# giltchcity/orb_slam3_ros

Measured on AMD Instinct MI355X. Metric: frames/sec ORB extract+match (752×480, 1000 kp) at 1/2/4/8 GPU; % HBM roofline, higher is better.
Workload: dtype u8; 1 GPU; EuRoC-MH01-like stereo 752x480 (BASELINE config 2): ORBextractor L+R (nFeatures=1000, scale 1.2, 8 levels, FAST 20/7) + ComputeStereoMatches; width=752, height=480, allgather=False, pipelines=1, parallelism=frame-sharded x1

## Files before the change

### orb_slam3_ros_amd/csrc/orbfe_kernels.hip

```cpp
#pragma clang fp contract(off)
#include <hip/hip_runtime.h>
#include <float.h>
#include <math.h>
#include <stdint.h>

#include <type_traits>

#include "brief_pattern.h"
#include "glibc_sincosf.h"
#include "orbfe_types.h"
#include "stl_sort.h"

namespace orbfe {

#define SYNC() __syncthreads()
#define WAVE_SYNC()                                               \
    do {                                                          \
        __builtin_amdgcn_fence(__ATOMIC_RELEASE, "workgroup");    \
        __builtin_amdgcn_s_waitcnt(0xc07f);                       \
        __builtin_amdgcn_wave_barrier();                          \
        __builtin_amdgcn_fence(__ATOMIC_ACQUIRE, "workgroup");    \
    } while (0)

__constant__ int c_umax[16] = {15, 15, 15, 15, 14, 14, 14, 13, 13, 12, 11, 10, 9, 8, 6, 3};
// ... 753 lines not shown
                    *(bi ? s_ent + pos : trash) = (uint16_t)((packed + i) | 0x4000 | (di << 15));
                    pos += (int)bi;
                }
                nent = __builtin_amdgcn_readlane(incl, 63);
            }
            WAVE_SYNC();
            for (int j0 = 0; j0 < nent; j0 += 128) {
                const int j = j0 + 2 * lane;
                const uint32_t e2 = j < nent ? ((const uint32_t*)s_ent)[j >> 1] : 0u;
                const bool ok0 = j < nent, ok1 = j + 1 < nent;
                const uint32_t e0 = e2 & 0xFFFFu, e1 = ok1 ? e2 >> 16 : e0;
                const uint8_t* q0 = s_px + (((e0 >> 7) & 127) + 3) * RS + (e0 & 127) + 3;
                const uint8_t* q1 = s_px + (((e1 >> 7) & 127) + 3) * RS + (e1 & 127) + 3;
                const orbfe_half2 v2 = as_h2(__builtin_bit_cast(uint32_t, orbfe_ushort2{q0[0], q1[0]}));
                const uint32_t bmask = ((e0 & 0x4000u) ? 0x00008000u : 0u) | ((e1 & 0x4000u) ? 0x80000000u : 0u);
                const orbfe_half2 ns = as_h2(0xBC00BC00u ^ bmask);
                const orbfe_half2 sv = as_h2(h2_bits(v2) ^ bmask);
                const uint8_t* t0 = q0 - 3 * RS - 3;
                const uint8_t* t1 = q1 - 3 * RS - 3;
                orbfe_half2 P[16];
#pragma unroll
                for (int k = 0; k < 16; k++) {
                    const int o = (kRingDy[k] + 3) * RS + kRingDx[k] + 3;
                    const orbfe_half2 x2 = as_h2(__builtin_bit_cast(uint32_t, orbfe_ushort2{t0[o], t1[o]}));
                    P[k] = __builtin_elementwise_fma(x2, ns, sv);
                }
                orbfe_half2 m3[16], m9[16];
#pragma unroll
                for (int k = 0; k < 16; k++) m3[k] = hmin(hmin(P[k], P[(k + 1) & 15]), P[(k + 2) & 15]);
#pragma unroll
                for (int k = 0; k < 16; k++) m9[k] = hmin(hmin(m3[k], m3[(k + 3) & 15]), m3[(k + 6) & 15]);
                orbfe_half2 r[6];
#pragma unroll
                for (int k = 0; k < 5; k++) r[k] = hmax(hmax(m9[3 * k], m9[3 * k + 1]), m9[3 * k + 2]);
                r[5] = m9[15];
                const orbfe_half2 mx = hmax(hmax(hmax(r[0], r[1]), r[2]), hmax(hmax(r[3], r[4]), r[5]));
                const uint32_t mb = h2_bits(mx);
                const int bx = (mb & 0x8000u) ? -1 : (int)(mb & 0x7fffu);
                const int by = (mb & 0x80000000u) ? -1 : (int)((mb >> 16) & 0x7fffu);
                const bool c0 = ok0 && bx > th, c1 = ok1 && by > th;
                if (c0) s_sc[(((e0 >> 7) & 127) + 1) * RS + (e0 & 127) + 1] = (uint8_t)(bx - 1);
                if (c1) s_sc[(((e1 >> 7) & 127) + 1) * RS + (e1 & 127) + 1] = (uint8_t)(by - 1);
                const int cc = (int)c0 + (int)c1;
                const unsigned long long b0 = __ballot(cc & 1), b1 = __ballot(cc & 2);
                int pos = ncorner + lanes_below(b0) + 2 * lanes_below(b1);
                if (c0) s_cor[pos++] = (uint16_t)(e0 & 0x3FFFu);
                if (c1) s_cor[pos] = (uint16_t)(e1 & 0x3FFFu);
                ncorner += __popcll(b0) + 2 * __popcll(b1);
            }
            WAVE_SYNC();
        }
        nsurv = 0;
        for (int i0 = 0; i0 < ncorner; i0 += 64) {
            const int i = i0 + lane;
            bool surv = false;
            int p = 0, sc = 0;
            if (i < ncorner) {
                p = s_cor[i];
                const uint8_t* q = s_sc + ((p >> 7) + 1) * RS + (p & 127) + 1;
                const int n0 = q[-RS - 1], n1 = q[-RS], n2 = q[-RS + 1], n3 = q[-1], n4 = q[1];
                const int n5 = q[RS - 1], n6 = q[RS], n7 = q[RS + 1];
                sc = q[0];
                const int mx = max(max(max(n0, n1), max(n2, n3)), max(max(n4, n5), max(n6, n7)));
                surv = sc > mx;
            }
            const unsigned long long m = __ballot(surv);
            if (surv)
                out[nsurv + lanes_below(m)] = (uint32_t)(xr0 + (p & 127)) | ((uint32_t)(yr0 + (p >> 7)) << 12) |
                                              ((uint32_t)sc << 24);
            nsurv += __popcll(m);
        }
        if (nsurv > 0) break;
        WAVE_SYNC();
    }
    if (lane == 0) cellcnt[(size_t)b * g.total_cells + c] = nsurv;
    WAVE_SYNC();
}

#define FAST_WPB 1
__global__ __launch_bounds__(64 * FAST_WPB) void k_fast(const uint8_t* const* imgs, int in_pitch, const uint8_t* pyr,
                                              int pyr_stride, OrbGeom g, FastLds fl, uint32_t* cellkeys,
                                              int* cellcnt, int c_lo, int c_hi, int cpw) {
    extern __shared__ __attribute__((aligned(16))) uint8_t smem_fast[];
    const int wave = __builtin_amdgcn_readfirstlane(threadIdx.x >> 6), lane = lane_id();
    const int lb = xcd_logical(block_linear(), gridDim.x * gridDim.y);
    const int bx = lb % gridDim.x, b = lb / gridDim.x;
    uint8_t* s_img = smem_fast + wave * fl.wave_bytes;
    uint8_t* s_sc = s_img + fl.roi;
    uint16_t* s_cor = (uint16_t*)(s_sc + fl.sc);
    uint16_t* s_ent = (uint16_t*)((uint8_t*)s_cor + fl.cor);
    const int cbeg = c_lo + (bx * FAST_WPB + wave) * cpw;
    if (cbeg >= c_hi) return;
    const int cend = min(cbeg + cpw, c_hi);
    orbfe_u32x4 pf[FAST_PF];
    FastCell cur = fast_cell(imgs, in_pitch, pyr, pyr_stride, g, b, cbeg);
    fast_prefetch(cur, lane, pf);
    for (int c = cbeg; c < cend; c++) {
        int ng, nd, cpr, rpl;
        fast_geom(cur, &ng, &nd, &cpr, &rpl);
        const int dw = cur.cols - 6, dh = cur.rows - 6;
        fast_stage_cell(cur, pf, s_img, s_sc, lane);
        const FastCell me = cur;
        if (c + 1 < cend) {
            cur = fast_cell_next(cur, imgs, in_pitch, pyr, pyr_stride, g, b);
            fast_prefetch(cur, lane, pf);
        }
        if (fast_rsd(nd) == 12)
            fast_cell_detect<12>(g, fl, me, ng, nd, dw, dh, s_img, s_sc, s_cor, s_ent, cellkeys, cellcnt, b, c, lane);
        else
            fast_cell_detect<0>(g, fl, me, ng, nd, dw, dh, s_img, s_sc, s_cor, s_ent, cellkeys, cellcnt, b, c, lane);
    }
}

#define OCT_NT 256
#define OCT_U 4
struct ExpLess64 {
    __device__ bool operator()(const unsigned long long& a, const unsigned long long& b) const {
        return (a >> 32) < (b >> 32);
    }
};
__device__ __forceinline__ int quadrant(uint32_t key, int x0, int x1, int y0, int y1) {
    const int halfX = (int)ceilf((float)(x1 - x0) / 2.f);
    const int halfY = (int)ceilf((float)(y1 - y0) / 2.f);
    const float fx = (float)(key & 0xfff), fy = (float)((key >> 12) & 0xfff);
    const int q = (fx < (float)(x0 + halfX)) ? (fy < (float)(y0 + halfY) ? 0 : 2) : (fy < (float)(y0 + halfY) ? 1 : 3);
    return q;
}
__device__ __forceinline__ void child_rect(int q, int x0, int x1, int y0, int y1, int* cx0, int* cx1, int* cy0,
                                           int* cy1) {
    const int mx = x0 + (int)ceilf((float)(x1 - x0) / 2.f);
    const int my = y0 + (int)ceilf((float)(y1 - y0) / 2.f);
    *cx0 = (q & 1) ? mx : x0;
    *cx1 = (q & 1) ? x1 : mx;
    *cy0 = (q & 2) ? my : y0;
    *cy1 = (q & 2) ? y1 : my;
}
template <int NT>
__device__ __forceinline__ int block_excl_scan(int* arr, int n, int* s_ws) {
    const int lane = lane_id(), wave = threadIdx.x >> 6;
    int carry = 0;
    for (int base = 0; base < n; base += NT) {
        const int i = base + threadIdx.x;
        const int v = i < n ? arr[i] : 0;
        const int incl = wave_incl_scan_dpp(v);
        if (lane == 63) s_ws[wave] = incl;
        SYNC();
        int woff = 0, tot = 0;
#pragma unroll
        for (int w = 0; w < NT / 64; w++) {
            const int t = s_ws[w];
            woff += w < wave ? t : 0;
            tot += t;
        }
        if (i < n) arr[i] = carry + woff + incl - v;
        carry += tot;
        SYNC();
    }
    return carry;
}

template <int NT>
__device__ __forceinline__ void block_scan2(int a, int b, int2* s_w2, int& exa, int& exb, int& tota, int& totb) {
    const int lane = lane_id(), wave = threadIdx.x >> 6;
    const int ia = wave_incl_scan_dpp(a), ib = wave_incl_scan_dpp(b);
    if (lane == 63) s_w2[wave] = make_int2(ia, ib);
    SYNC();
    int oa = 0, ob = 0, ta = 0, tb = 0;
#pragma unroll
    for (int w = 0; w < NT / 64; w++) {
        const int2 t = s_w2[w];
        oa += w < wave ? t.x : 0;
        ob += w < wave ? t.y : 0;
        ta += t.x;
        tb += t.y;
    }
    exa = oa + ia - a;
    exb = ob + ib - b;
    tota = ta;
    totb = tb;
}

__device__ __forceinline__ int wave_scan_lds(int* arr, int n) {
    const int lane = lane_id();
    int carry = 0;
    for (int base = 0; base < n; base += 64) {
        const int i = base + lane;
        const int v = i < n ? arr[i] : 0;
        const int incl = wave_incl_scan_dpp(v);
        if (i < n) arr[i] = carry + incl - v;
        carry += __builtin_amdgcn_readlane(incl, 63);
    }
    WAVE_SYNC();
    return carry;
}

__device__ __forceinline__ void atomic_inc_runs(int* base, int t, bool act) {
    const int lane = lane_id();
    const int key = act ? t : -1 - lane;
    const int prev = __builtin_amdgcn_update_dpp(INT_MIN, key, 0x138, 0xf, 0xf, false);
    const bool head = key != prev;
    const unsigned long long hm = __ballot(head);
    const unsigned long long above = hm & ~((2ull << lane) - 1ull);
    const int next = above ? (int)__builtin_ctzll(above) : 64;
    if (head && act) atomicAdd(&base[t], next - lane);
}

__device__ __forceinline__ int wave_partition(unsigned long long* a, int lo, int hi, int* lpos, int* rpos) {
    const int tid = lane_id();
    const unsigned long long lt = (1ull << tid) - 1ull;
    unsigned long long xpiv;
    {
        const int ia = lo + 1, ib = lo + (hi - lo) / 2, ic = hi - 1;
        const unsigned long long x0 = a[lo], xa = a[ia], xb = a[ib], xc = a[ic];
        const ExpLess64 comp;
        int pick;
        if (comp(xa, xb)) pick = comp(xb, xc) ? ib : (comp(xa, xc) ? ic : ia);
        else pick = comp(xa, xc) ? ia : (comp(xb, xc) ? ic : ib);
        xpiv = pick == ia ? xa : (pick == ib ? xb : xc);
        if (tid == 0) {
            a[lo] = xpiv;
            a[pick] = x0;
        }
    }
    WAVE_SYNC();
    const unsigned P = (unsigned)(xpiv >> 32);
    const int m = hi - lo - 1;
    int* lp = lpos + lo;
    int* rp = rpos + lo;
    int nl = 0, nr = 0;
    for (int b0 = 0; b0 < m; b0 += 64) {
        const int i = b0 + tid;
        bool lf = false, rf = false;
        if (i < m) {
            lf = !((unsigned)(a[lo + 1 + i] >> 32) < P);
            rf = !(P < (unsigned)(a[hi - 1 - i] >> 32));
        }
        const unsigned long long lm = __ballot(lf), rm = __ballot(rf);
        if (lf) lp[nl + __popcll(lm & lt)] = lo + 1 + i;
        if (rf) rp[nr + __popcll(rm & lt)] = hi - 1 - i;
        nl += __popcll(lm);
        nr += __popcll(rm);
    }
    WAVE_SYNC();
    const int kmax = min(nl, nr);
    int sw = 0;
    for (int b0 = 0; b0 < kmax; b0 += 64) {
        const int k = b0 + tid;
        sw += __popcll(__ballot(k < kmax && lp[k] < rp[k]));
    }
    for (int k = tid; k < sw; k += 64) {
        const unsigned long long x = a[lp[k]];
        a[lp[k]] = a[rp[k]];
        a[rp[k]] = x;
    }
    int cut;
    if (sw == 0) cut = lp[0];
    else cut = (sw < nl && lp[sw] < rp[sw - 1]) ? lp[sw] : rp[sw - 1];
    WAVE_SYNC();
    return cut;
}

__device__ __forceinline__ void wave_leaf(unsigned long long* a, int lo, int hi) {
    const int lane = lane_id();
    const int len = hi - lo;
    if (len <= 1) return;
    if (len > 16) {
        if (lane == 0) st_heap_sort(a + lo, len, ExpLess64());
        WAVE_SYNC();
        return;
    }
    const unsigned long long x = a[lo + min(lane, len - 1)];
    const unsigned kx = (unsigned)(x >> 32);
    int r = 0;
#pragma unroll
    for (int u = 0; u < 16; u++) {
        const unsigned ku = (unsigned)__builtin_amdgcn_readlane((int)kx, u);
        r += (u < len && (ku < kx || (ku == kx && u < lane))) ? 1 : 0;
    }
    WAVE_SYNC();
    if (lane < len) a[lo + r] = x;
    WAVE_SYNC();
}

#if ORBFE_OCT_STAMPS
__device__ unsigned long long g_sort_ts[16 * 16 + 16];
__shared__ unsigned long long s_dbg_ts[16 * 16 + 16];
#endif
__device__ __forceinline__ unsigned long long rl64(unsigned long long x, int l) {
    const unsigned lo = (unsigned)__builtin_amdgcn_readlane((int)(unsigned)x, l);
    const unsigned hi = (unsigned)__builtin_amdgcn_readlane((int)(unsigned)(x >> 32), l);
    return ((unsigned long long)hi << 32) | lo;
}
__device__ __forceinline__ unsigned long long bp64(unsigned long long x, int src) {
    const unsigned lo = (unsigned)__builtin_amdgcn_ds_bpermute(src << 2, (int)(unsigned)x);
    const unsigned hi = (unsigned)__builtin_amdgcn_ds_bpermute(src << 2, (int)(unsigned)(x >> 32));
    return ((unsigned long long)hi << 32) | lo;
}
__device__ __forceinline__ unsigned long long pm64(unsigned long long x, int dst) {
    const unsigned lo = (unsigned)__builtin_amdgcn_ds_permute(dst << 2, (int)(unsigned)x);
    const unsigned hi = (unsigned)__builtin_amdgcn_ds_permute(dst << 2, (int)(unsigned)(x >> 32));
    return ((unsigned long long)hi << 32) | lo;
}

__device__ __forceinline__ void wave_sort64(unsigned long long* a, int lo0, int len, int d0) {
    const int lane = lane_id();
#if ORBFE_OCT_STAMPS
    int s64i = 0;
#define S64_STAMP() do { if (lane == 0 && s64i < 15 && (threadIdx.x >> 6) == 0 && blockIdx.x == 0 && blockIdx.y == 0) s_dbg_ts[256 + s64i] = __builtin_amdgcn_s_memtime(); s64i++; } while (0)
#else
#define S64_STAMP() do { } while (0)
#endif
    S64_STAMP();
    unsigned long long x = a[lo0 + min(lane, len - 1)];
    const unsigned long long below = (1ull << lane) - 1ull;
    const unsigned long long above = lane == 63 ? 0ull : (~0ull << (lane + 1));
    unsigned long long leafm = 0, heapm = 0;
    int sg_lo = 0, sg_hi = lane == 0 ? len : 0, sg_dp = lane == 0 ? d0 : 0;
    int sp = 1;
    while (sp > 0) {
        --sp;
        const int lo = __builtin_amdgcn_readlane(sg_lo, sp), hi = __builtin_amdgcn_readlane(sg_hi, sp);
        const int dp = __builtin_amdgcn_readlane(sg_dp, sp);
        if (hi - lo <= 16 || dp == 0) {
            leafm |= 1ull << lo;
            if (hi - lo > 16) heapm |= 1ull << lo;
            continue;
        }
        const int ia = lo + 1, ib = lo + (hi - lo) / 2, ic = hi - 1;
        const unsigned kx = (unsigned)(x >> 32);
        const unsigned ka = (unsigned)__builtin_amdgcn_readlane((int)kx, ia);
        const unsigned kb = (unsigned)__builtin_amdgcn_readlane((int)kx, ib);
        const unsigned kc = (unsigned)__builtin_amdgcn_readlane((int)kx, ic);
        int pick;
        if (ka < kb) pick = kb < kc ? ib : (ka < kc ? ic : ia);
        else pick = ka < kc ? ia : (kb < kc ? ic : ib);
        const unsigned long long x0 = rl64(x, lo), xp = rl64(x, pick);
        if (lane == lo) x = xp;
        else if (lane == pick) x = x0;
        const unsigned P = (unsigned)(xp >> 32);
        const unsigned k = (unsigned)(x >> 32);
        const bool inr = lane > lo && lane < hi;
        const bool lf = inr && !(k < P), rf = inr && !(P < k);
        const unsigned long long LM = __ballot(lf), RM = __ballot(rf);
        const int rl = __popcll(LM & below), rr = __popcll(RM & above);
        const bool sL = lf && __popcll(RM & above) > rl;
        const int sw = __popcll(__ballot(sL));
        const bool sR = rf && rr < sw;
        int cut;
        if (sw == 0) {
            cut = __builtin_ctzll(LM);
        } else {
            const int rp = __builtin_ctzll(__ballot(rf && rr == sw - 1));
            const int lp = sw < __popcll(LM) ? __builtin_ctzll(__ballot(lf && rl == sw)) : 64;
            cut = lp < rp ? lp : rp;
            const unsigned long long vR = pm64(x, sR ? rr : 63);
            const unsigned long long vL = pm64(x, sL ? rl : 63);
            const unsigned long long fromR = bp64(vR, rl & 63), fromL = bp64(vL, rr & 63);
            if (sL) x = fromR;
            else if (sR) x = fromL;
        }
        if (lane == sp) { sg_lo = cut; sg_hi = hi; sg_dp = dp - 1; }
        if (lane == sp + 1) { sg_lo = lo; sg_hi = cut; sg_dp = dp - 1; }
        sp += 2;
        S64_STAMP();
    }
    S64_STAMP();
    const unsigned long long upto = leafm & ~above;
    const int ls = 63 - __builtin_clzll(upto | 1ull);
    const unsigned long long after = leafm & above;
    const int le = after ? __builtin_ctzll(after) : len;
    const bool heap = (heapm >> ls) & 1ull;
    const unsigned kx = (unsigned)(x >> 32);
    unsigned kj[16];
#pragma unroll
    for (int u = 0; u < 16; u++) kj[u] = (unsigned)__builtin_amdgcn_ds_bpermute(min(ls + u, 63) << 2, (int)kx);
    int r = 0;
#pragma unroll
    for (int u = 0; u < 16; u++) {
        const int j = ls + u;
        r += (int)((j < le) & ((kj[u] < kx) | ((kj[u] == kx) & (j < lane))));
    }
    x = pm64(x, (lane < len && !heap) ? ls + r : lane);
    if (lane < len) a[lo0 + lane] = x;
    if (heapm) {
        WAVE_SYNC();
        if (lane == 0) {
            unsigned long long hm = heapm;
            while (hm) {
                const int hs = __builtin_ctzll(hm);
                hm &= hm - 1ull;
                const unsigned long long nx = leafm & (hs == 63 ? 0ull : (~0ull << (hs + 1)));
                const int he = nx ? __builtin_ctzll(nx) : len;
                st_heap_sort(a + lo0 + hs, he - hs, ExpLess64());
            }
        }
    }
    WAVE_SYNC();
    S64_STAMP();
#if ORBFE_OCT_STAMPS
    if (lane == 0 && (threadIdx.x >> 6) == 0 && blockIdx.x == 0 && blockIdx.y == 0) s_dbg_ts[256 + 15] = s64i;
#endif
#undef S64_STAMP
}

__device__ __forceinline__ void wave_sort_seg(unsigned long long* a, int lo0, int hi0, int dp0, int* lpos, int* rpos) {
    const int tid = lane_id();
    int sg_lo = lo0, sg_hi = tid == 0 ? hi0 : 0, sg_dp = tid == 0 ? dp0 : 0;
    int sp = 1;
    while (sp > 0) {
        --sp;
        const int lo = __builtin_amdgcn_readlane(sg_lo, sp), hi = __builtin_amdgcn_readlane(sg_hi, sp);
        const int depth = __builtin_amdgcn_readlane(sg_dp, sp);
        if (hi - lo <= 64 && depth > 0) {
            if (hi - lo > 1) wave_sort64(a, lo, hi - lo, depth);
            continue;
        }
        if (depth == 0) {
            wave_leaf(a, lo, hi);
            continue;
        }
        const int cut = wave_partition(a, lo, hi, lpos, rpos);
        if (tid == sp) { sg_lo = cut; sg_hi = hi; sg_dp = depth - 1; }
        if (tid == sp + 1) { sg_lo = lo; sg_hi = cut; sg_dp = depth - 1; }
        sp += 2;
    }
}

__device__ __forceinline__ unsigned long long seg_pack(int lo, int hi, int d) {
    return (unsigned long long)(unsigned)lo | ((unsigned long long)(unsigned)hi << 16) | ((unsigned long long)d << 32);
}

__device__ __forceinline__ void block_introsort(unsigned long long* a, int n, int* fl, int* lpos, int* rpos, int* leaves,
                                unsigned long long* tmp, int4* segs, int* s_ws, int* s_ctl) {
    (void)fl; (void)leaves; (void)segs; (void)s_ws;
    const int lane = lane_id(), wave = threadIdx.x >> 6, nw = blockDim.x >> 6;
#if ORBFE_OCT_STAMPS
    int sti = 0;
#define SORT_STAMP() do { if (lane == 0 && sti < 15 && blockIdx.x == 0 && blockIdx.y == 0) s_dbg_ts[wave * 16 + sti] = __builtin_amdgcn_s_memtime(); sti++; } while (0)
#else
#define SORT_STAMP() do { } while (0)
#endif
    SORT_STAMP();
    if (threadIdx.x == 0) {
        tmp[0] = seg_pack(0, n, 2 * st_lg(n));
#pragma unroll
        for (int k = 0; k < 8; k++) s_ctl[k] = 0;
    }
    SYNC();
    SORT_STAMP();
    if (n <= 1) return;
    unsigned long long* cur = tmp;
    unsigned long long* nxt = tmp + 2 * nw;
    int S = 1, r = 0;
    while (S > 0 && S < nw && r < 7) {
        bool any = false;
        for (int s = wave; s < S; s += nw) {
            const unsigned long long e = cur[s];
            const int lo = (int)(e & 0xffff), hi = (int)((e >> 16) & 0xffff), d = (int)(e >> 32);
            unsigned long long c0 = 0, c1 = 0;
            if (hi - lo <= 16 || d == 0) {
                wave_leaf(a, lo, hi);
            } else if (hi - lo <= 64) {
                wave_sort64(a, lo, hi - lo, d);
            } else {
                const int cut = wave_partition(a, lo, hi, lpos, rpos);
                if (hi - cut <= 16 || d == 1) wave_leaf(a, cut, hi);
                else c0 = seg_pack(cut, hi, d - 1);
                if (cut - lo <= 16 || d == 1) wave_leaf(a, lo, cut);
                else c1 = seg_pack(lo, cut, d - 1);
            }
            if (lane == 0) {
                nxt[2 * s] = c0;
                nxt[2 * s + 1] = c1;
            }
            any = any || c0 != 0 || c1 != 0;
        }
        if (any && lane == 0) s_ctl[r] = 1;
        SYNC();
        SORT_STAMP();
        S = s_ctl[r] ? 2 * S : 0;
        r++;
        unsigned long long* t = cur; cur = nxt; nxt = t;
    }
    for (int s = wave; s < S; s += nw) {
        const unsigned long long e = cur[s];
        if (e) wave_sort_seg(a, (int)(e & 0xffff), (int)((e >> 16) & 0xffff), (int)(e >> 32), lpos, rpos);
    }
    SORT_STAMP();
    SYNC();
    SORT_STAMP();
#if ORBFE_OCT_STAMPS
    if (lane == 0 && blockIdx.x == 0 && blockIdx.y == 0) s_dbg_ts[wave * 16 + 15] = sti;
    SYNC();
    if (blockIdx.x == 0 && blockIdx.y == 0)
        for (int i = threadIdx.x; i < 16 * 16 + 16; i += blockDim.x) g_sort_ts[i] = s_dbg_ts[i];
#endif
#undef SORT_STAMP
}

__global__ __launch_bounds__(OCT_NT) void k_debug_block_sort(unsigned long long* a, int n) {
    extern __shared__ __attribute__((aligned(16))) uint8_t smem_dbs[];
    unsigned long long* la = (unsigned long long*)smem_dbs;
    unsigned long long* tmp = la + n;
    int* fl = (int*)(tmp + n);
    int* lpos = fl + n;
    int* rpos = lpos + n;
    int* leaves = rpos + n;
    int4* segs = (int4*)(((uintptr_t)(leaves + n) + 15) & ~(uintptr_t)15);
    __shared__ int s_ws[OCT_NT / 64];
    __shared__ int s_ctl[8];
    for (int i = threadIdx.x; i < n; i += OCT_NT) la[i] = a[i];
    SYNC();
    block_introsort(la, n, fl, lpos, rpos, leaves, tmp, segs, s_ws, s_ctl);
    for (int i = threadIdx.x; i < n; i += OCT_NT) a[i] = la[i];
}

template <int NT>
__global__ __launch_bounds__(NT, NT <= 256 ? 6 : 1) void k_octree(OrbGeom g, const uint32_t* __restrict__ cellkeys,
                                                   const int* __restrict__ cellcnt, uint32_t* lkeys,
                                                   uint16_t* nodeof, uint32_t* outkeys, int* lvinfo, int* ranks,
                                                   const int2* __restrict__ laps, unsigned long long* tstamp,
                                                   int lv0) {
    extern __shared__ __attribute__((aligned(16))) uint8_t smem_oct[];
    const int b = blockIdx.x, l = lv0 + (int)blockIdx.y, tid = threadIdx.x;
    const int lap0 = laps[b].x, lap1 = laps[b].y;
    const OrbLevel& L = g.lv[l];
    const int NC = g.node_cap;
    const int ncell = L.n_cols * L.n_rows;
    uint8_t* p = smem_oct;
    auto carve = [&](size_t bytes) { uint8_t* r = p; p += (bytes + 15) & ~(size_t)15; return r; };
    int* cellpre = (int*)carve(sizeof(int) * (g.max_cells_level + 1));
    int16_t *Cx0 = (int16_t*)carve(2 * NC), *Cx1 = (int16_t*)carve(2 * NC);
    int16_t *Cy0 = (int16_t*)carve(2 * NC), *Cy1 = (int16_t*)carve(2 * NC);
    int* Csz = (int*)carve(4 * NC);
    int16_t *Xx0 = (int16_t*)carve(2 * NC), *Xx1 = (int16_t*)carve(2 * NC);
    int16_t *Xy0 = (int16_t*)carve(2 * NC), *Xy1 = (int16_t*)carve(2 * NC);
    int* Xsz = (int*)carve(4 * NC);
    int* Ccnt = (int*)carve(16 * NC);
    int* Xcnt = (int*)carve(16 * NC);
    int16_t* childpos = (int16_t*)carve(8 * NC);
    int16_t* newpos = (int16_t*)carve(2 * NC);
    int* divorder = (int*)carve(4 * NC);
    int* tmpA = (int*)carve(4 * NC);
    int* tmpB = (int*)carve(4 * NC);
    int* tmpC = (int*)carve(4 * NC);
    int* procp = (int*)carve(4 * NC);
    unsigned long long* expv = (unsigned long long*)carve(8 * NC);
    int4* segs = (int4*)carve(sizeof(int4) * ORBFE_SORT_STACK);
    __shared__ int s_ws[NT / 64];
    __shared__ int s_misc[8];
    __shared__ int2 s_ws2[NT / 64];

    unsigned long long* ts = (tstamp && b == 0) ? tstamp + 64 * l : nullptr;
    int tsi = 0;
    (void)ts;
    (void)tsi;
#if ORBFE_OCT_STAMPS
    __shared__ unsigned long long s_octts[64];
#define OCT_STAMP() do { if (ts && tid == 0 && tsi < 62) s_octts[tsi] = __builtin_amdgcn_s_memtime(); tsi++; } while (0)
#else
#define OCT_STAMP() do { } while (0)
#endif
    OCT_STAMP();
    const int* cc = cellcnt + (size_t)b * g.total_cells + L.cell_base;
    for (int i = tid; i < ncell; i += NT) cellpre[i] = cc[i];
    SYNC();
    const int K = block_excl_scan<NT>(cellpre, ncell, s_ws);
    if (tid == 0) cellpre[ncell] = K;
    const int nIni = L.n_ini;
    const float hX = L.hx;
    const int H = (L.h - ORBFE_MINB) - ORBFE_MINB;
    const bool fini = NT >= 1024 && K <= NT * (NT >= 1024 ? 8 : OCT_U) && nIni <= NT;
    for (int i = tid; i < nIni; i += NT) tmpA[i] = 0;
    if (fini)
        for (int i = tid; i < 4 * nIni; i += NT) tmpC[i] = 0;
    for (int i = tid; i < 4 * NC; i += NT) Ccnt[i] = 0;
    SYNC();
    const size_t kbase = (size_t)b * g.cellkeys_per_img + L.cellkey_off;
    uint32_t* keys = lkeys + kbase;
    uint16_t* nof = nodeof + kbase;
    const uint32_t* ck = cellkeys + kbase;
    constexpr int OU = NT >= 1024 ? 8 : OCT_U;
    const bool regk = NT >= 1024 && K <= NT * OU;
    uint32_t rkv[OU];
    int rq[OU];
    for (int kb = 0; kb < K; kb += NT * OU) {
        const int k0 = kb + tid;
        uint32_t v[OU];
#pragma unroll
        for (int u = 0; u < OU; u++) {
            if ((u & 3) == 0 && kb + NT * u >= K) break;
            const int k = min(k0 + NT * u, K - 1);
            int lo = 0, hi = ncell - 1;
            while (lo < hi) {
                const int mid = (lo + hi + 1) >> 1;
                if (cellpre[mid] <= k) lo = mid; else hi = mid - 1;
            }
            v[u] = ck[(size_t)lo * L.cell_cap + (k - cellpre[lo])];
        }
#pragma unroll
        for (int u = 0; u < OU; u++) {
            if ((u & 3) == 0 && kb + NT * u >= K) break;
            if (regk) rkv[u] = v[u];
            else if (k0 + NT * u < K) keys[k0 + NT * u] = v[u];
            const int col = (int)((float)(v[u] & 0xfff) / hX);
            atomic_inc_runs(tmpA, col, k0 + NT * u < K);
            if (fini) {
                rq[u] = col;
                atomic_inc_runs(tmpC, 4 * col + quadrant(v[u], (int)(hX * (float)col), (int)(hX * (float)(col + 1)), 0, H),
                                k0 + NT * u < K);
            }
        }
    }
    OCT_STAMP();
    SYNC();
    int n;
    if (fini) {
        const int i = tid;
        const bool f = i < nIni && tmpA[i] > 0;
        int ex, exZ, totZ;
        block_scan2<NT>(f ? 1 : 0, 0, s_ws2, ex, exZ, n, totZ);
        (void)exZ;
        (void)totZ;
        if (f) {
            Cx0[ex] = (int16_t)(int)(hX * (float)i);
            Cx1[ex] = (int16_t)(int)(hX * (float)(i + 1));
            Cy0[ex] = 0;
            Cy1[ex] = (int16_t)H;
            Csz[ex] = tmpA[i];
            *(int4*)&Ccnt[4 * ex] = *(const int4*)&tmpC[4 * i];
        }
        if (i < nIni) tmpB[i] = ex;
        for (int j = tid; j < NC; j += NT) divorder[j] = -1;
        SYNC();
#pragma unroll
        for (int u = 0; u < (NT >= 1024 ? 8 : OCT_U); u++) {
            if ((u & 3) == 0 && NT * u >= K) break;
            rq[u] = tmpB[rq[u]];
        }
        OCT_STAMP();
    } else {
    for (int i = tid; i < nIni; i += NT) tmpB[i] = tmpA[i] > 0 ? 1 : 0;
    SYNC();
    n = block_excl_scan<NT>(tmpB, nIni, s_ws);
    for (int i = tid; i < nIni; i += NT) {
        if (tmpA[i] > 0) {
            const int q = tmpB[i];
            Cx0[q] = (int16_t)(int)(hX * (float)i);
            Cx1[q] = (int16_t)(int)(hX * (float)(i + 1));
            Cy0[q] = 0;
            Cy1[q] = (int16_t)H;
            Csz[q] = tmpA[i];
        }
    }
    SYNC();
    for (int kb = 0; kb < K; kb += NT * OU) {
        const int k0 = kb + tid;
        uint32_t v[OU];
#pragma unroll
        for (int u = 0; u < OU; u++) v[u] = regk ? rkv[u] : keys[min(k0 + NT * u, K - 1)];
#pragma unroll
        for (int u = 0; u < OU; u++) {
            if ((u & 3) == 0 && kb + NT * u >= K) break;
            const int k = k0 + NT * u;
            const uint32_t key = v[u];
            const int q = tmpB[(int)((float)(key & 0xfff) / hX)];
            if (regk) rq[u] = q;
            else if (k < K) nof[k] = (uint16_t)q;
            atomic_inc_runs(Ccnt, 4 * q + quadrant(key, Cx0[q], Cx1[q], Cy0[q], Cy1[q]), k < K && Csz[q] > 1);
        }
    }
    for (int i = tid; i < NC; i += NT) divorder[i] = -1;
    SYNC();
    OCT_STAMP();
    }

    const int N = L.budget;
    bool phase2 = false, finish = false;
    int m = 0;
    int guard = 0;
    while (!finish && guard++ < 100000) {
        const int prevN = n;
        int newN, Etot;
        if (!phase2 && n <= NT) {
            const int i = tid;
            const bool live = i < n;
            const int csz = live ? Csz[i] : 0;
            const bool div = csz > 1;
            int4 cq = make_int4(0, 0, 0, 0);
            if (div) cq = *(const int4*)&Ccnt[4 * i];
            const int cv[4] = {cq.x, cq.y, cq.z, cq.w};
            int c = 0, e = 0;
#pragma unroll
            for (int k = 0; k < 4; k++) { c += cv[k] > 0; e += cv[k] > 1; }
            int exA, exB, totA, totB;
            block_scan2<NT>(live ? (div ? 1 : 0x10000) : 0, c | (e << 16), s_ws2, exA, exB, totA, totB);
            const int Ctot = totB & 0xffff;
            Etot = totB >> 16;
            newN = Ctot + (totA >> 16);
            if (div) {
                divorder[i] = exA & 0xffff;
                const int start = Ctot - ((exB & 0xffff) + c);
                int kk = 0;
                const int px0 = Cx0[i], px1 = Cx1[i], py0 = Cy0[i], py1 = Cy1[i];
                int cpos[4];
#pragma unroll
                for (int ch = 3; ch >= 0; ch--) {
                    const int v = cv[ch];
                    cpos[ch] = -1;
                    if (v > 0) {
                        const int np = start + kk++;
                        cpos[ch] = np;
                        childpos[4 * i + ch] = (int16_t)np;
                        int a0, a1, b0, b1;
                        child_rect(ch, px0, px1, py0, py1, &a0, &a1, &b0, &b1);
                        Xx0[np] = (int16_t)a0; Xx1[np] = (int16_t)a1;
                        Xy0[np] = (int16_t)b0; Xy1[np] = (int16_t)b1;
                        Xsz[np] = v;
                    } else {
                        childpos[4 * i + ch] = -1;
                    }
                }
                int ei = exB >> 16;
#pragma unroll
                for (int ch = 0; ch < 4; ch++) {
                    const int v = cv[ch];
                    if (v > 1) {
                        int a0, a1, b0, b1;
                        child_rect(ch, px0, px1, py0, py1, &a0, &a1, &b0, &b1);
                        expv[ei] = ((unsigned long long)v << 44) | ((unsigned long long)(a0 & 0xfff) << 32) |
                                   (unsigned long long)(uint16_t)cpos[ch];
                        ei++;
                    }
                }
            } else if (live) {
                divorder[i] = -1;
                const int np = Ctot + (exA >> 16);
                newpos[i] = (int16_t)np;
                Xx0[np] = Cx0[i]; Xx1[np] = Cx1[i];
                Xy0[np] = Cy0[i]; Xy1[np] = Cy1[i];
                Xsz[np] = csz;
            }
            for (int j = tid; j < 4 * newN; j += NT) Xcnt[j] = 0;
            SYNC();
            OCT_STAMP();
        } else if (phase2 && m <= NT && n <= NT) {
#if ORBFE_OCT_STAMPS
            if (ts && tid == 0) s_octts[62] = (unsigned long long)m | ((unsigned long long)n << 16) | ((unsigned long long)K << 32);
#endif
            block_introsort(expv, m, tmpC, tmpA, tmpB, Xcnt + 2 * NC, (unsigned long long*)Xcnt, segs, s_ws,
                            s_misc);
            OCT_STAMP();
            const int t = tid;
            const bool live = t < m;
            int q = 0;
            int4 cq = make_int4(0, 0, 0, 0);
            if (live) {
                q = (int)(expv[m - 1 - t] & 0xffffffffull);
                cq = *(const int4*)&Ccnt[4 * q];
            }
            const int cv[4] = {cq.x, cq.y, cq.z, cq.w};
            int c = 0, e = 0;
#pragma unroll
            for (int k = 0; k < 4; k++) { c += cv[k] > 0; e += cv[k] > 1; }
            const int grow = live ? c - 1 : 0;
            if (tid == 0) s_misc[6] = m;
            int exG, exCE, totG, totCE;
            block_scan2<NT>(grow, c | (e << 16), s_ws2, exG, exCE, totG, totCE);
            if (live && n + exG + grow >= N) atomicMin(&s_misc[6], t + 1);
            if (live) tmpB[t] = exCE + (c | (e << 16));
            SYNC();
            const int T_div = s_misc[6];
            const int tot = T_div > 0 ? tmpB[T_div - 1] : 0;
            const int Ctot = tot & 0xffff;
            Etot = tot >> 16;
            if (t < T_div) {
                divorder[q] = t;
                const int start = Ctot - ((exCE & 0xffff) + c);
                int kk = 0;
                const int px0 = Cx0[q], px1 = Cx1[q], py0 = Cy0[q], py1 = Cy1[q];
                int cpos[4];
#pragma unroll
                for (int ch = 3; ch >= 0; ch--) {
                    const int v = cv[ch];
                    cpos[ch] = -1;
                    if (v > 0) {
                        const int np = start + kk++;
                        cpos[ch] = np;
                        childpos[4 * q + ch] = (int16_t)np;
                        int a0, a1, b0, b1;
                        child_rect(ch, px0, px1, py0, py1, &a0, &a1, &b0, &b1);
                        Xx0[np] = (int16_t)a0; Xx1[np] = (int16_t)a1;
                        Xy0[np] = (int16_t)b0; Xy1[np] = (int16_t)b1;
                        Xsz[np] = v;
                    } else {
                        childpos[4 * q + ch] = -1;
                    }
                }
                int ei = exCE >> 16;
#pragma unroll
                for (int ch = 0; ch < 4; ch++) {
                    const int v = cv[ch];
                    if (v > 1) {
                        int a0, a1, b0, b1;
                        child_rect(ch, px0, px1, py0, py1, &a0, &a1, &b0, &b1);
                        expv[ei] = ((unsigned long long)v << 44) | ((unsigned long long)(a0 & 0xfff) << 32) |
                                   (unsigned long long)(uint16_t)cpos[ch];
                        ei++;
                    }
                }
            }
            SYNC();
            const int i = tid;
            const bool keep = i < n && divorder[i] < 0;
            int exK, exZ, nKeep, totZ;
            block_scan2<NT>(keep ? 1 : 0, 0, s_ws2, exK, exZ, nKeep, totZ);
            (void)exZ;
            (void)totZ;
            if (keep) {
                const int np = Ctot + exK;
                newpos[i] = (int16_t)np;
                Xx0[np] = Cx0[i]; Xx1[np] = Cx1[i];
                Xy0[np] = Cy0[i]; Xy1[np] = Cy1[i];
                Xsz[np] = Csz[i];
            }
            newN = Ctot + nKeep;
            for (int j = tid; j < 4 * newN; j += NT) Xcnt[j] = 0;
            SYNC();
            OCT_STAMP();
        } else {
            int T_div;
            if (!phase2) {
                for (int i = tid; i < n; i += NT) tmpA[i] = Csz[i] > 1 ? 1 : 0;
                SYNC();
                for (int i = tid; i < n; i += NT) divorder[i] = Csz[i] > 1 ? 1 : -1;
                T_div = block_excl_scan<NT>(tmpA, n, s_ws);
                for (int i = tid; i < n; i += NT)
                    if (divorder[i] >= 0) { divorder[i] = tmpA[i]; procp[tmpA[i]] = i; }
                SYNC();
            } else {
#if ORBFE_OCT_STAMPS
                if (ts && tid == 0) s_octts[62] = (unsigned long long)m | ((unsigned long long)n << 16) | ((unsigned long long)K << 32);
#endif
                block_introsort(expv, m, tmpC, tmpA, tmpB, Xcnt + 2 * NC, (unsigned long long*)Xcnt, segs, s_ws,
                                s_misc);
                OCT_STAMP();
                for (int t = tid; t < m; t += NT) {
                    const int q = (int)(expv[m - 1 - t] & 0xffffffffull);
                    const int4 cq = *(const int4*)&Ccnt[4 * q];
                    tmpA[t] = (cq.x > 0) + (cq.y > 0) + (cq.z > 0) + (cq.w > 0) - 1;
                    procp[t] = q;
                }
                if (tid == 0) s_misc[6] = m;
                SYNC();
                (void)block_excl_scan<NT>(tmpA, m, s_ws);
                for (int t = tid; t < m; t += NT) {
                    const int q = procp[t];
                    const int4 cq = *(const int4*)&Ccnt[4 * q];
                    const int grow = (cq.x > 0) + (cq.y > 0) + (cq.z > 0) + (cq.w > 0) - 1;
                    if (n + tmpA[t] + grow >= N) atomicMin(&s_misc[6], t + 1);
                }
                SYNC();
                T_div = s_misc[6];
                for (int t = tid; t < T_div; t += NT) divorder[procp[t]] = t;
                SYNC();
            }
            OCT_STAMP();
            for (int t = tid; t < T_div; t += NT) {
                const int q = procp[t];
                int c = 0, e = 0;
                const int4 cq = *(const int4*)&Ccnt[4 * q];
                const int cv[4] = {cq.x, cq.y, cq.z, cq.w};
    #pragma unroll
                for (int k = 0; k < 4; k++) { c += cv[k] > 0; e += cv[k] > 1; }
                tmpB[t] = c;
                tmpC[t] = e;
            }
            SYNC();
            const int Ctot = block_excl_scan<NT>(tmpB, T_div, s_ws);
            Etot = block_excl_scan<NT>(tmpC, T_div, s_ws);
            for (int t = tid; t < T_div; t += NT) {
                const int q = procp[t];
                const int4 cq = *(const int4*)&Ccnt[4 * q];
                const int cv[4] = {cq.x, cq.y, cq.z, cq.w};
                int c = 0;
    #pragma unroll
                for (int k = 0; k < 4; k++) c += cv[k] > 0;
                const int start = Ctot - (tmpB[t] + c);
                int kk = 0;
                const int px0 = Cx0[q], px1 = Cx1[q], py0 = Cy0[q], py1 = Cy1[q];
                int cpos[4];
    #pragma unroll
                for (int ch = 3; ch >= 0; ch--) {
                    const int v = cv[ch];
                    cpos[ch] = -1;
                    if (v > 0) {
                        const int np = start + kk++;
                        cpos[ch] = np;
                        childpos[4 * q + ch] = (int16_t)np;
                        int a0, a1, b0, b1;
                        child_rect(ch, px0, px1, py0, py1, &a0, &a1, &b0, &b1);
                        Xx0[np] = (int16_t)a0; Xx1[np] = (int16_t)a1;
                        Xy0[np] = (int16_t)b0; Xy1[np] = (int16_t)b1;
                        Xsz[np] = v;
                    } else {
                        childpos[4 * q + ch] = -1;
                    }
                }
                int e = tmpC[t];
    #pragma unroll
                for (int ch = 0; ch < 4; ch++) {
                    const int v = cv[ch];
                    if (v > 1) {
                        int a0, a1, b0, b1;
                        child_rect(ch, px0, px1, py0, py1, &a0, &a1, &b0, &b1);
                        expv[e] = ((unsigned long long)v << 44) | ((unsigned long long)(a0 & 0xfff) << 32) |
                                  (unsigned long long)(uint16_t)cpos[ch];
                        e++;
                    }
                }
            }
            for (int i = tid; i < n; i += NT) tmpA[i] = divorder[i] < 0 ? 1 : 0;
            SYNC();
            const int nKeep = block_excl_scan<NT>(tmpA, n, s_ws);
            for (int i = tid; i < n; i += NT) {
                if (divorder[i] < 0) {
                    const int np = Ctot + tmpA[i];
                    newpos[i] = (int16_t)np;
                    Xx0[np] = Cx0[i]; Xx1[np] = Cx1[i];
                    Xy0[np] = Cy0[i]; Xy1[np] = Cy1[i];
                    Xsz[np] = Csz[i];
                }
            }
            newN = Ctot + nKeep;
            for (int i = tid; i < 4 * newN; i += NT) Xcnt[i] = 0;
            SYNC();
            OCT_STAMP();
        }
        for (int kb = 0; kb < K; kb += NT * OU) {
            const int k0 = kb + tid;
            uint32_t v[OU];
            int qv[OU];
#pragma unroll
            for (int u = 0; u < OU; u++) {
                const int k = min(k0 + NT * u, K - 1);
                v[u] = regk ? rkv[u] : keys[k];
                qv[u] = regk ? rq[u] : nof[k];
            }
#pragma unroll
            for (int u = 0; u < OU; u++) {
                if ((u & 3) == 0 && kb + NT * u >= K) break;
                const int k = k0 + NT * u;
                const uint32_t key = v[u];
                const int q = qv[u];
                int np;
                if (divorder[q] >= 0) np = childpos[4 * q + quadrant(key, Cx0[q], Cx1[q], Cy0[q], Cy1[q])];
                else np = newpos[q];
                if (regk) rq[u] = np;
                else if (k < K) nof[k] = (uint16_t)np;
                atomic_inc_runs(Xcnt, 4 * np + quadrant(key, Xx0[np], Xx1[np], Xy0[np], Xy1[np]), k < K && Xsz[np] > 1);
            }
        }
        SYNC();
        for (int i = tid; i < NC; i += NT) divorder[i] = -1;
        {
            int16_t* t;
            int* ti;
            t = Cx0; Cx0 = Xx0; Xx0 = t; t = Cx1; Cx1 = Xx1; Xx1 = t;
            t = Cy0; Cy0 = Xy0; Xy0 = t; t = Cy1; Cy1 = Xy1; Xy1 = t;
            ti = Csz; Csz = Xsz; Xsz = ti; ti = Ccnt; Ccnt = Xcnt; Xcnt = ti;
        }
        n = newN;
        m = Etot;
        if (n > NC - 4) { n = NC - 4; finish = true; }
        if (n >= N || n == prevN) finish = true;
        else if (!phase2 && n + 3 * m > N) phase2 = true;
    }
    OCT_STAMP();
    unsigned long long* best = (unsigned long long*)Xcnt;
    for (int i = tid; i < n; i += NT) best[i] = 0ull;
    SYNC();
    for (int k0 = tid; k0 < K; k0 += NT * OU) {
        uint32_t v[OU];
        int qv[OU];
#pragma unroll
        for (int u = 0; u < OU; u++) {
            const int k = min(k0 + NT * u, K - 1);
            v[u] = regk ? rkv[u] : keys[k];
            qv[u] = regk ? rq[u] : nof[k];
        }
#pragma unroll
        for (int u = 0; u < OU; u++) {
            const int k = k0 + NT * u;
            if ((u & 3) == 0 && k0 - tid + NT * u >= K) break;
            if (k < K)
                atomicMax(&best[qv[u]], ((unsigned long long)(v[u] >> 24) << 32) | (0xFFFFFFFFull - (unsigned)k));
        }
    }
    SYNC();
    uint32_t* ok = outkeys + (size_t)b * g.out_per_img + L.out_off;
    int* rk = ranks + (size_t)b * g.out_per_img + L.out_off;
    auto emit = [&](int i, uint32_t key) {
        const int x = (int)(key & 0xfff) + ORBFE_MINB, y = (int)((key >> 12) & 0xfff) + ORBFE_MINB;
        ok[i] = (uint32_t)x | ((uint32_t)y << 12) | (key & 0xff000000u);
        const float sx = (l == 0) ? (float)x : (float)x * L.scale;
        tmpA[i] = (sx >= (float)lap0 && sx <= (float)lap1) ? 1 : 0;
    };
    if (regk) {
#pragma unroll
        for (int u = 0; u < OU; u++) {
            const int k = tid + NT * u;
            if ((u & 3) == 0 && NT * u >= K) break;
            if (k < K && best[rq[u]] == (((unsigned long long)(rkv[u] >> 24) << 32) | (0xFFFFFFFFull - (unsigned)k)))
                emit(rq[u], rkv[u]);
        }
    } else {
        for (int i = tid; i < n; i += NT) emit(i, keys[0xFFFFFFFFu - (unsigned)(best[i] & 0xFFFFFFFFull)]);
    }
    SYNC();
    int nlap, nmono;
    if (n <= NT) {
        const int f = tid < n ? tmpA[tid] : 0;
        int exl, exm;
        block_scan2<NT>(f, tid < n ? 1 - f : 0, s_ws2, exl, exm, nlap, nmono);
        if (tid < n) rk[tid] = f ? (int)(0x40000000 | exl) : exm;
    } else {
        for (int i = tid; i < n; i += NT) tmpB[i] = 1 - tmpA[i];
        SYNC();
        nlap = block_excl_scan<NT>(tmpA, n, s_ws);
        nmono = block_excl_scan<NT>(tmpB, n, s_ws);
        for (int i = tid; i < n; i += NT) {
            const bool lap = (i + 1 < n ? tmpA[i + 1] : nlap) != tmpA[i];
            rk[i] = lap ? (int)(0x40000000 | tmpA[i]) : tmpB[i];
        }
    }
    OCT_STAMP();
#if ORBFE_OCT_STAMPS
    if (ts && tid == 0) {
        for (int i = 0; i < min(tsi, 62); i++) ts[i] = s_octts[i];
        ts[62] = s_octts[62];
        ts[63] = (unsigned long long)tsi;
    }
#endif
#undef OCT_STAMP
    if (tid == 0) {
        int* inf = lvinfo + ((size_t)b * g.nlevels + l) * 4;
        inf[0] = n; inf[1] = nlap; inf[2] = nmono; inf[3] = K;
    }
}

__device__ __forceinline__ float fast_atan2_dev(float y, float x) {
    const float p1 = 0.9997878412794807f * (float)(180 / M_PI);
    const float p3 = -0.3258083974640975f * (float)(180 / M_PI);
    const float p5 = 0.1555786518463281f * (float)(180 / M_PI);
    const float p7 = -0.04432655554792128f * (float)(180 / M_PI);
    const float ax = fabsf(x), ay = fabsf(y);
    float a, c, c2;
    if (ax >= ay) {
        c = ay / (ax + (float)DBL_EPSILON);
        c2 = c * c;
        a = (((p7 * c2 + p5) * c2 + p3) * c2 + p1) * c;
    } else {
        c = ax / (ay + (float)DBL_EPSILON);
        c2 = c * c;
        a = 90.f - (((p7 * c2 + p5) * c2 + p3) * c2 + p1) * c;
    }
    if (x < 0) a = 180.f - a;
    if (y < 0) a = 360.f - a;
    return a;
}

#define DP_R 21
#define DP_N (2 * DP_R + 1)
#define DP_RAW_S 48
#define DP_NP 22
#define DP_P_S 40
#define DP_WAVE_LDS 5600
#define DP_ND (DP_N * (DP_RAW_S / 4))
struct DescSlot {
    int valid, l, x, y, interior, pitch, gx0, sh;
    int border;
    uint32_t key;
    size_t o;
    gptr_u8 im;
};
struct DescImg {
    int n, lap_before, mono_before;
    int ntot, mono_tot;
};
__device__ __forceinline__ int row_incl_scan_dpp(int v) {
    v += __builtin_amdgcn_update_dpp(0, v, 0x111, 0xf, 0xf, false);
    v += __builtin_amdgcn_update_dpp(0, v, 0x112, 0xf, 0xf, false);
    v += __builtin_amdgcn_update_dpp(0, v, 0x114, 0xf, 0xf, false);
    v += __builtin_amdgcn_update_dpp(0, v, 0x118, 0xf, 0xf, false);
    return v;
}
__device__ __forceinline__ DescImg desc_img(const OrbGeom& g, const int* __restrict__ inf, int lane) {
    int4 li = make_int4(0, 0, 0, 0);
    if (lane < g.nlevels) li = ((const int4*)inf)[lane];
    DescImg di;
    di.n = li.x;
    const int lapi = row_incl_scan_dpp(li.y), monoi = row_incl_scan_dpp(li.z), ni = row_incl_scan_dpp(li.x);
    di.lap_before = lapi - li.y;
    di.mono_before = monoi - li.z;
    di.ntot = __builtin_amdgcn_readlane(ni, 15);
    di.mono_tot = __builtin_amdgcn_readlane(monoi, 15);
    return di;
}
__device__ __forceinline__ DescSlot desc_slot(const uint8_t* const* imgs, int in_pitch, const uint8_t* pyr,
                                              int pyr_stride, const OrbGeom& g, const DescImg& di, uint32_t kv,
                                              int rv, int j, int* lvl, int b, int flat) {
    DescSlot d;
    d.valid = 0;
    if (flat >= g.out_per_img) return d;
    int l = *lvl;
    while (l + 1 < g.nlevels && flat >= g.lv[l + 1].out_off) l++;
    *lvl = l;
    const OrbLevel& L = g.lv[l];
    if (flat - L.out_off >= __builtin_amdgcn_readlane(di.n, l)) return d;
    d.valid = 1;
    d.l = l;
    d.key = (uint32_t)__builtin_amdgcn_readlane((int)kv, j);
    d.x = d.key & 0xfff;
    d.y = (d.key >> 12) & 0xfff;
    const int rk = __builtin_amdgcn_readlane(rv, j);
    const int slot = (rk & 0x40000000) ? di.ntot - 1 - (__builtin_amdgcn_readlane(di.lap_before, l) + (rk & 0x3fffffff))
                                       : __builtin_amdgcn_readlane(di.mono_before, l) + rk;
    d.o = (size_t)b * g.kp_cap + slot;
    d.im = level_base(imgs, in_pitch, pyr, pyr_stride, g, b, l, &d.pitch);
    const int px0 = d.x - DP_R, py0 = d.y - DP_R;
    d.gx0 = px0 & ~3;
    d.sh = px0 - d.gx0;
    const bool aligned = (d.pitch & 3) == 0 && ((((uintptr_t)d.im) & 3) == 0);
    d.interior = px0 >= 0 && py0 >= 0 && py0 + DP_N <= L.h && d.gx0 + DP_RAW_S + 4 <= L.w && aligned;
    d.border = 0;
    if (!d.interior && aligned && d.pitch >= DP_RAW_S) {
        const int ws = min(max(d.gx0, 0), d.pitch - DP_RAW_S);
        const int s = px0 - ws;
        const int nl = max(-px0, 0), cr = min(L.w - px0, DP_N);
        if (py0 > -L.h && py0 + DP_N < 2 * L.h && nl <= 8 && DP_N - cr <= 8 && 2 * nl < cr &&
            2 * cr - DP_N - 1 >= nl && nl + s >= 0 && cr + s <= DP_RAW_S) {
            d.border = 1 | (((s >> 2) + 2) << 1) | (nl << 4) | ((DP_N - cr) << 8) | (L.h << 12);
            d.gx0 = ws;
            d.sh = s & 3;
        }
    }
    return d;
}
__device__ __forceinline__ void desc_load(const DescSlot& d, int lane, orbfe_u32x4 (&q)[3]) {
    const int r0 = small_div(lane, 3), k = lane - 3 * r0;
    if (d.border) {
        gptr_u8 b0 = d.im + d.gx0 + 16 * k;
#pragma unroll
        for (int u = 0; u < 3; u++) {
            const uint32_t row = (uint32_t)reflect101(d.y - DP_R + min(r0 + 21 * u, DP_N - 1), d.border >> 12);
            q[u] = *(const ORBFE_GLOBAL orbfe_u32x4*)(b0 + __umul24(row, (uint32_t)d.pitch));
        }
        return;
    }
// ... 642 lines not shown
```

Baseline: 162,100 frames/s.

## Partially sort octree expansion candidates using histogram-derived top-R bound

Before sorting the octree node expansion list, a 64-bucket histogram over the high key bits is built with atomics. A reverse scan of it finds how many of the largest entries can be consumed before the feature target N is reached. The introsort then skips segments lying entirely below that cutoff and leaves them unsorted, and the later scan and division loops run only over R entries instead of m. This cuts sort and scan work in the distribution phase, at the cost of an extra histogram pass and a reused shared buffer. Correctness relies on the bucket bound being conservative.

```diff
diff --git a/orb_slam3_ros_amd/csrc/orbfe_kernels.hip b/orb_slam3_ros_amd/csrc/orbfe_kernels.hip
--- a/orb_slam3_ros_amd/csrc/orbfe_kernels.hip
+++ b/orb_slam3_ros_amd/csrc/orbfe_kernels.hip
@@ -1079,7 +1079,7 @@
     return ((unsigned long long)hi << 32) | lo;
 }
 
-__device__ __forceinline__ void wave_sort64(unsigned long long* a, int lo0, int len, int d0) {
+__device__ __forceinline__ void wave_sort64(unsigned long long* a, int lo0, int len, int d0, int keep) {
     const int lane = lane_id();
 #if ORBFE_OCT_STAMPS
     int s64i = 0;
@@ -1092,12 +1092,19 @@
     const unsigned long long below = (1ull << lane) - 1ull;
     const unsigned long long above = lane == 63 ? 0ull : (~0ull << (lane + 1));
     unsigned long long leafm = 0, heapm = 0;
+    unsigned long long skipm = 0;
+    const int kp = keep - lo0;
     int sg_lo = 0, sg_hi = lane == 0 ? len : 0, sg_dp = lane == 0 ? d0 : 0;
     int sp = 1;
     while (sp > 0) {
         --sp;
         const int lo = __builtin_amdgcn_readlane(sg_lo, sp), hi = __builtin_amdgcn_readlane(sg_hi, sp);
         const int dp = __builtin_amdgcn_readlane(sg_dp, sp);
+        if (hi <= kp) {
+            leafm |= 1ull << lo;
+            skipm |= 1ull << lo;
+            continue;
+        }
         if (hi - lo <= 16 || dp == 0) {
             leafm |= 1ull << lo;
             if (hi - lo > 16) heapm |= 1ull << lo;
@@ -1146,7 +1153,7 @@
     const int ls = 63 - __builtin_clzll(upto | 1ull);
     const unsigned long long after = leafm & above;
     const int le = after ? __builtin_ctzll(after) : len;
-    const bool heap = (heapm >> ls) & 1ull;
+    const bool heap = ((heapm | skipm) >> ls) & 1ull;
     const unsigned kx = (unsigned)(x >> 32);
     unsigned kj[16];
 #pragma unroll
@@ -1180,7 +1187,8 @@
 #undef S64_STAMP
 }
 
-__device__ __forceinline__ void wave_sort_seg(unsigned long long* a, int lo0, int hi0, int dp0, int* lpos, int* rpos) {
+__device__ __forceinline__ void wave_sort_seg(unsigned long long* a, int lo0, int hi0, int dp0, int* lpos, int* rpos,
+                                              int keep) {
     const int tid = lane_id();
     int sg_lo = lo0, sg_hi = tid == 0 ? hi0 : 0, sg_dp = tid == 0 ? dp0 : 0;
     int sp = 1;
@@ -1188,8 +1196,9 @@
         --sp;
         const int lo = __builtin_amdgcn_readlane(sg_lo, sp), hi = __builtin_amdgcn_readlane(sg_hi, sp);
         const int depth = __builtin_amdgcn_readlane(sg_dp, sp);
+        if (hi <= keep) continue;
         if (hi - lo <= 64 && depth > 0) {
-            if (hi - lo > 1) wave_sort64(a, lo, hi - lo, depth);
+            if (hi - lo > 1) wave_sort64(a, lo, hi - lo, depth, keep);
             continue;
         }
         if (depth == 0) {
@@ -1208,7 +1217,8 @@
 }
 
 __device__ __forceinline__ void block_introsort(unsigned long long* a, int n, int* fl, int* lpos, int* rpos, int* leaves,
-                                unsigned long long* tmp, int4* segs, int* s_ws, int* s_ctl) {
+                                unsigned long long* tmp, int4* segs, int* s_ws, int* s_ctl,
+                                const int* headp = nullptr) {
     (void)fl; (void)leaves; (void)segs; (void)s_ws;
     const int lane = lane_id(), wave = threadIdx.x >> 6, nw = blockDim.x >> 6;
 #if ORBFE_OCT_STAMPS
@@ -1226,6 +1236,7 @@
     SYNC();
     SORT_STAMP();
     if (n <= 1) return;
+    const int keep = headp ? n - *headp : 0;
     unsigned long long* cur = tmp;
     unsigned long long* nxt = tmp + 2 * nw;
     int S = 1, r = 0;
@@ -1238,12 +1249,13 @@
             if (hi - lo <= 16 || d == 0) {
                 wave_leaf(a, lo, hi);
             } else if (hi - lo <= 64) {
-                wave_sort64(a, lo, hi - lo, d);
+                wave_sort64(a, lo, hi - lo, d, keep);
             } else {
                 const int cut = wave_partition(a, lo, hi, lpos, rpos);
                 if (hi - cut <= 16 || d == 1) wave_leaf(a, cut, hi);
                 else c0 = seg_pack(cut, hi, d - 1);
-                if (cut - lo <= 16 || d == 1) wave_leaf(a, lo, cut);
+                if (cut <= keep) { }
+                else if (cut - lo <= 16 || d == 1) wave_leaf(a, lo, cut);
                 else c1 = seg_pack(lo, cut, d - 1);
             }
             if (lane == 0) {
@@ -1261,7 +1273,7 @@
     }
     for (int s = wave; s < S; s += nw) {
         const unsigned long long e = cur[s];
-        if (e) wave_sort_seg(a, (int)(e & 0xffff), (int)((e >> 16) & 0xffff), (int)(e >> 32), lpos, rpos);
+        if (e) wave_sort_seg(a, (int)(e & 0xffff), (int)((e >> 16) & 0xffff), (int)(e >> 32), lpos, rpos, keep);
     }
     SORT_STAMP();
     SYNC();
@@ -1290,6 +1302,26 @@
     SYNC();
     block_introsort(la, n, fl, lpos, rpos, leaves, tmp, segs, s_ws, s_ctl);
     for (int i = threadIdx.x; i < n; i += OCT_NT) a[i] = la[i];
+}
+
+template <int NT>
+__device__ __forceinline__ void octree_walk_bound(const unsigned long long* expv, int m, const int* Ccnt, int n, int N,
+                                                  int* hist) {
+    for (int t = threadIdx.x; t < m; t += NT) {
+        const unsigned long long e = expv[t];
+        const int4 cq = *(const int4*)&Ccnt[4 * (int)(e & 0xffffffffull)];
+        const int grow = (cq.x > 0) + (cq.y > 0) + (cq.z > 0) + (cq.w > 0) - 1;
+        atomicAdd(&hist[min((int)(e >> 44), 63)], 1 | (grow << 16));
+    }
+    SYNC();
+    if (threadIdx.x < 64) {
+        const int lane = lane_id();
+        const int incl = wave_incl_scan_dpp(hist[63 - lane]);
+        hist[63 - lane] = 0;
+        const unsigned long long ok = __ballot(n + (incl >> 16) >= N);
+        const int R = ok ? (__builtin_amdgcn_readlane(incl, (int)__builtin_ctzll(ok)) & 0xffff) : m;
+        if (lane == 0) hist[64] = R;
+    }
 }
 
 template <int NT>
@@ -1324,6 +1356,7 @@
     int* procp = (int*)carve(4 * NC);
     unsigned long long* expv = (unsigned long long*)carve(8 * NC);
     int4* segs = (int4*)carve(sizeof(int4) * ORBFE_SORT_STACK);
+    int* whist = (int*)segs;
     __shared__ int s_ws[NT / 64];
     __shared__ int s_misc[8];
     __shared__ int2 s_ws2[NT / 64];
@@ -1349,6 +1382,7 @@
     const int H = (L.h - ORBFE_MINB) - ORBFE_MINB;
     const bool fini = NT >= 1024 && K <= NT * (NT >= 1024 ? 8 : OCT_U) && nIni <= NT;
     for (int i = tid; i < nIni; i += NT) tmpA[i] = 0;
+    if (tid < 64) whist[tid] = 0;
     if (fini)
         for (int i = tid; i < 4 * nIni; i += NT) tmpC[i] = 0;
     for (int i = tid; i < 4 * NC; i += NT) Ccnt[i] = 0;
@@ -1525,11 +1559,14 @@
 #if ORBFE_OCT_STAMPS
             if (ts && tid == 0) s_octts[62] = (unsigned long long)m | ((unsigned long long)n << 16) | ((unsigned long long)K << 32);
 #endif
+            const bool part = m > 16;
+            if (part) octree_walk_bound<NT>(expv, m, Ccnt, n, N, whist);
             block_introsort(expv, m, tmpC, tmpA, tmpB, Xcnt + 2 * NC, (unsigned long long*)Xcnt, segs, s_ws,
-                            s_misc);
+                            s_misc, part ? whist + 64 : nullptr);
             OCT_STAMP();
+            const int R = part ? whist[64] : m;
             const int t = tid;
-            const bool live = t < m;
+            const bool live = t < R;
             int q = 0;
             int4 cq = make_int4(0, 0, 0, 0);
             if (live) {
@@ -1541,7 +1578,7 @@
 #pragma unroll
             for (int k = 0; k < 4; k++) { c += cv[k] > 0; e += cv[k] > 1; }
             const int grow = live ? c - 1 : 0;
-            if (tid == 0) s_misc[6] = m;
+            if (tid == 0) s_misc[6] = R;
             int exG, exCE, totG, totCE;
             block_scan2<NT>(grow, c | (e << 16), s_ws2, exG, exCE, totG, totCE);
             if (live && n + exG + grow >= N) atomicMin(&s_misc[6], t + 1);
@@ -1619,19 +1656,22 @@
 #if ORBFE_OCT_STAMPS
                 if (ts && tid == 0) s_octts[62] = (unsigned long long)m | ((unsigned long long)n << 16) | ((unsigned long long)K << 32);
 #endif
+                const bool part = m > 16;
+                if (part) octree_walk_bound<NT>(expv, m, Ccnt, n, N, whist);
                 block_introsort(expv, m, tmpC, tmpA, tmpB, Xcnt + 2 * NC, (unsigned long long*)Xcnt, segs, s_ws,
-                                s_misc);
+                                s_misc, part ? whist + 64 : nullptr);
                 OCT_STAMP();
-                for (int t = tid; t < m; t += NT) {
+                const int R = part ? whist[64] : m;
+                for (int t = tid; t < R; t += NT) {
                     const int q = (int)(expv[m - 1 - t] & 0xffffffffull);
                     const int4 cq = *(const int4*)&Ccnt[4 * q];
                     tmpA[t] = (cq.x > 0) + (cq.y > 0) + (cq.z > 0) + (cq.w > 0) - 1;
                     procp[t] = q;
                 }
-                if (tid == 0) s_misc[6] = m;
+                if (tid == 0) s_misc[6] = R;
                 SYNC();
-                (void)block_excl_scan<NT>(tmpA, m, s_ws);
-                for (int t = tid; t < m; t += NT) {
+                (void)block_excl_scan<NT>(tmpA, R, s_ws);
+                for (int t = tid; t < R; t += NT) {
                     const int q = procp[t];
                     const int4 cq = *(const int4*)&Ccnt[4 * q];
                     const int grow = (cq.x > 0) + (cq.y > 0) + (cq.z > 0) + (cq.w > 0) - 1;
```

Result: no change. 162,000 frames/s (-0.0%).
